# penn-graphics-research/HOT

Measured on AMD Instinct MI355X. Metric: ms per nonlinear (L-BFGS) iteration; P2G+G2P Mparticles/s; achieved HBM GB/s vs roofline, lower is better.
Workload: dtype f64; 1 GPU; C2: one 63^3-cell cube x 8 ppc (63^3 cells per GPU), fixed-corotated E=50000 nu=0.3, dx=0.01, dt=1/24, -lsolver 3 -mg_level 3 -smoother 5 -coarseSolver 2 --project --linesearch --bcproject --usecn -cneps 1e-7; particles_per_gpu=2000376, particles_total=2000376, nodes_total=267601, levels=3, parallelism=1 GPU

## Files before the change

### hot_amd/binding.py

```python
import ctypes as C
import numpy as np

_DT = {0: np.float32, 1: np.float64}


class hot_config(C.Structure):
    _fields_ = [
        ("dtype", C.c_int32), ("device", C.c_int32), ("dx", C.c_double), ("gravity", C.c_double * 3),
        ("apic_rpic_ratio", C.c_double), ("cfl", C.c_double), ("lsolver", C.c_int32), ("Ainv", C.c_int32),
        ("smoother", C.c_int32), ("coarseSolver", C.c_int32), ("levelCnt", C.c_int32), ("times", C.c_int32),
        ("levelscale", C.c_int32), ("omega", C.c_double), ("topomega", C.c_double), ("cneps", C.c_double),
        ("useCN", C.c_int32), ("project", C.c_int32), ("systemBCProject", C.c_int32), ("linesearch", C.c_int32),
        ("matrixFree", C.c_int32), ("boundaryType", C.c_int32), ("useAdaptiveHessian", C.c_int32),
        ("topDownMGS", C.c_int32), ("max_iterations", C.c_int32), ("plasticity", C.c_int32),
        ("yield_stress", C.c_double), ("snow", C.c_double * 5), ("profile", C.c_int32), ("debug_store", C.c_int32), ("useBaselineMultigrid", C.c_int32), ("gs_chain", C.c_int32), ("gs_sub_block", C.c_int32), ("shard_gs", C.c_int32), ("shard_replicated", C.c_int32), ("ls_energy_only", C.c_int32), ("linear_iteration_cap", C.c_int32), ("shard_owner", C.c_int32), ("deterministic", C.c_int32), ("reserved", C.c_int32 * 4),
    ]


class hot_collision_object(C.Structure):
    _fields_ = [("shape", C.c_int32), ("type", C.c_int32), ("p0", C.c_double * 3), ("p1", C.c_double * 3), ("friction", C.c_double),
                ("b", C.c_double * 3), ("dbdt", C.c_double * 3), ("R", C.c_double * 9), ("omega", C.c_double * 3), ("s", C.c_double), ("dsdt", C.c_double), ("lsq", C.c_double * 4)]


STICKY, SLIP, SEPARATE = 1, 2, 3
# ... 13 lines not shown
        ("iterations", C.c_int32), ("converged", C.c_int32), ("linesearch_trials", C.c_int32),
        ("linear_iterations", C.c_int32), ("vcycles", C.c_int32), ("dropped_pairs", C.c_int32),
        ("num_nodes", C.c_int32), ("num_levels", C.c_int32), ("final_scaled_residual", C.c_double),
        ("energy", C.c_double), ("ms_sort", C.c_double), ("ms_p2g", C.c_double), ("ms_begin", C.c_double),
        ("ms_hessian", C.c_double), ("ms_mg_build", C.c_double), ("ms_solve", C.c_double), ("ms_g2p", C.c_double),
        ("ms_total", C.c_double), ("comm_calls", C.c_int64), ("comm_bytes_index", C.c_int64), ("comm_bytes_data", C.c_int64), ("comm_calls_index", C.c_int64),
    ]

    def as_dict(self):
        return {k: getattr(self, k) for k, _ in self._fields_}


ABI_SYMBOLS = [
    "default_config", "create", "destroy", "last_error", "sync", "set_particles", "get_particles", "sort",
    "get_counts", "get_indexing", "p2g", "get_grid", "set_bc", "set_sticky_halfspaces", "set_collision_objects", "begin_step", "get_dv",
    "set_dv", "update_state", "get_particle_state", "residual", "project", "cn_tolerance", "build_hessian",
    "matfree_multiply", "build_mg", "get_level", "get_matrix", "get_level_nnzb", "get_prolongation", "spmv", "restrict", "prolong",
    "smooth", "vcycle", "solve", "g2p", "line_search", "should_exit", "recover_solution", "transform_residual", "compute_step", "write_partio", "write_restart", "read_restart", "set_particle_ids", "get_particle_ids", "get_stream", "set_comm", "constitutive_eval", "plasticity_eval", "advance", "calculate_dt", "advance_frame", "profile_reset", "profile_count", "profile_get", "version", "abi_version",
]
ABI_VERSION = 7


PRODUCT_ONLY_SYMBOLS = ["rccl_unique_id", "rccl_attach", "rccl_selftest", "get_level_inblock_nnzb", "copy_bandwidth",
                        "set_plasticity_classes", "get_plasticity_classes", "plasticity_eval_classes"]


class HotError(RuntimeError):
    pass


def _ptr(a):
    if a is None:
        return None
    if hasattr(a, "data_ptr"):
        return C.c_void_p(a.data_ptr())
    return C.c_void_p(a.ctypes.data)


class HotLib:
    def __init__(self, path, prefix="hot_"):
        self.path = str(path)
        self.prefix = prefix
        self.lib = C.CDLL(self.path)
        vp, i32, i64, dbl = C.c_void_p, C.c_int32, C.c_int64, C.c_double
        P = C.POINTER
        sig = {
            "default_config": (None, [P(hot_config)]),
# ... 538 lines not shown
```

### hot_amd/csrc/hot_impl.h

```cpp
#pragma once
#include "hot_ctx.h"
#include <atomic>
#include <functional>

namespace hot {

template <class T>
struct GsImg {
    static constexpr size_t hdr_elems = 2 * 64 * 9;
    static constexpr size_t cap_entries = 1340 + 1;
    static constexpr size_t per_dir = cap_entries * 9, per_block = hdr_elems + 2 * per_dir;
    static constexpr size_t idx_per_dir = 64 * 64;
};

struct GsPlan {
    enum Path {
        CHAINED,
        COLOUR,
        PAIR,
        PER_COLOUR,
        SIMPLE,
    } path;
    int sb;
    int nmerge;
    bool winv;
    bool marks;
};
struct GsBuild {
    bool winv;
    bool images;
    bool colour_lists;
};

template <class T>
__host__ __device__ inline int home_rank(const uint64_t* split, int R, int x, int y, int z, int level)
{
    using G = Geo<T>;
    const uint64_t page = G::linear_offset((x & ~3) << level, (y & ~3) << level, (z & ~3) << level) >> 12;
    int r = 0;
    while (r < R - 1 && page >= split[r]) ++r;
    return r;
}

template <class T>
struct Level {
    int n = 0;
    int id = 0;
    bool built = false;
    long long nnzb = 0;
// ... 536 lines not shown
```

### hot_amd/csrc/mg_gs.hip

```cpp
#include "hot_impl.h"

namespace hot {

#ifdef HOT_AB_KERNELS
#include "ab_src/mg_gs_ab1.hip"
#endif

template <class T, int SB>
struct GsLds {
    static constexpr int TRI = SB * (SB - 1) / 2 + 1;
    static constexpr size_t bytes = (size_t)9 * TRI * sizeof(T) + SB * 3 * sizeof(T) + 5 * SB * sizeof(int32_t);
};
template <class T>
struct GsWinv {
    static constexpr int img_elems = (9 * GsLds<T, 64>::TRI + 15) / 16 * 16;
};
template <int SB>
__device__ __forceinline__ int gs_tri_fwd(int row, int colm) { return (SB - 1) * colm - (colm * (colm - 1)) / 2 + (row - colm - 1); }
__device__ __forceinline__ int gs_tri_bwd(int row, int colm) { return (colm * (colm - 1)) / 2 + row; }
template <bool FWD>
__device__ __forceinline__ int gs_winv_idx(int row, int colm) { return FWD ? (row * (row - 1)) / 2 + colm : ((63 - row) * (62 - row)) / 2 + (63 - colm); }

template <class T>
__device__ __forceinline__ void gs_store_tri(T* tri, int TRI, int idx, const T* __restrict__ di, const T (&b)[9])
// ... 660 lines not shown
{
    const size_t i = (size_t)blockIdx.x * blockDim.x + threadIdx.x;
    if (i >= n) return;
    if constexpr (sizeof(T) == 8)
        ((unsigned long long*)x)[i] = GsUnset<double>::bits;
    else
        ((unsigned*)x)[i] = GsUnset<float>::bits;
}
struct GsPasses {
    int npass;
    int wg_begin[34];
    int block0[33];
    int sub[33];
    int color[33];
};

#ifdef HOT_GS_CLOCKS
__device__ unsigned long long gs_clk[34 * 8];
#define GS_CLK(i) \
    do { \
        const unsigned long long t_ = clock64(); \
        gclk_[i] += t_ - gt0_, gt0_ = t_; \
    } while (0)
#else
#define GS_CLK(i)
#endif
template <class T, bool FWD, int SB, bool WINV = false>
__global__ __launch_bounds__(SB * 16) void k_gs_sweep(const int32_t* __restrict__ col, const T* __restrict__ val, const uint32_t* __restrict__ ckey, const int32_t* __restrict__ gs_order,
    const int32_t* __restrict__ block_start, const T* __restrict__ diagVal, const T* __restrict__ diagBlockInv, const T* __restrict__ rhs, T* x, T* hD, GsPasses P,
    const int32_t* __restrict__ rowcnt, int* err ,
    T* unset_next ,
    const T* __restrict__ gs_w )
{
    extern __shared__ __attribute__((aligned(16))) char gs_smem[];
    constexpr int TRI = GsLds<T, SB>::TRI;
    static_assert(!WINV || SB == 64, "the inverse images are whole-block images");
#ifdef HOT_GS_CLOCKS
    unsigned long long gclk_[5] = { 0, 0, 0, 0, 0 }, gt0_ = clock64();
#endif
    constexpr int RQ = 4, NW = SB / RQ;
    auto ld3 = [&](int64_t j, T& x0, T& x1, T& x2) {
        x0 = __hip_atomic_load(x + 3 * j, __ATOMIC_RELAXED, __HIP_MEMORY_SCOPE_AGENT), x1 = __hip_atomic_load(x + 3 * j + 1, __ATOMIC_RELAXED, __HIP_MEMORY_SCOPE_AGENT),
        x2 = __hip_atomic_load(x + 3 * j + 2, __ATOMIC_RELAXED, __HIP_MEMORY_SCOPE_AGENT);
        int spins = 0;
        while (GsUnset<T>::is(x0) || GsUnset<T>::is(x1) || GsUnset<T>::is(x2)) {
            __builtin_amdgcn_s_sleep(2);
            if (++spins > (1 << 21) || ((spins & 1023) == 0 && *(volatile int*)err)) {
                *(volatile int*)err = 1;
                break;
            }
            x0 = __hip_atomic_load(x + 3 * j, __ATOMIC_RELAXED, __HIP_MEMORY_SCOPE_AGENT), x1 = __hip_atomic_load(x + 3 * j + 1, __ATOMIC_RELAXED, __HIP_MEMORY_SCOPE_AGENT),
            x2 = __hip_atomic_load(x + 3 * j + 2, __ATOMIC_RELAXED, __HIP_MEMORY_SCOPE_AGENT);
        }
    };
    T* tri = (T*)gs_smem;
    T* sv = tri + (WINV ? GsWinv<T>::img_elems : 9 * TRI);
    int32_t* nodes = (int32_t*)(sv + 3 * SB);
    const int tid = threadIdx.x, lane = tid & 63, w = tid >> 6;
    int p = 0;
    while (p + 1 < P.npass && (int)blockIdx.x >= P.wg_begin[p + 1]) ++p;
    const int b = P.block0[p] + ((int)blockIdx.x - P.wg_begin[p]);
    const int lo = P.sub[p] * SB;
    const int start = block_start[b] + lo, cnt = max(0, min(SB, block_start[b + 1] - start));
    int32_t* rng = nodes + SB;
    T* sDinv = (T*)(nodes + 5 * SB);
    T* sD = sDinv + 9 * SB;
    T* srhs = sD + 9 * SB;
    if (!WINV)
        for (int e = tid; e < 9 * TRI; e += 64 * NW) tri[e] = (T)0;
    if (tid < SB) nodes[tid] = tid < cnt ? gs_order[start + tid] : -1;
    __syncthreads();
    GS_CLK(0);
    if (WINV) {
        constexpr int IMG_BYTES = GsWinv<T>::img_elems * (int)sizeof(T);
        const char* wg = (const char*)(gs_w + ((size_t)b * 2 + (FWD ? 0 : 1)) * GsWinv<T>::img_elems);
        for (int c = w; c * 1024 < IMG_BYTES; c += NW) {
            const int off = c * 1024 + lane * 16;
            if (off < IMG_BYTES)
                __builtin_amdgcn_global_load_lds((const __attribute__((address_space(1))) void*)(wg + off), (__attribute__((address_space(3))) void*)((char*)tri + c * 1024), 16, 0, 0);
        }
    }
    for (int e = tid; e < 9 * cnt; e += 64 * NW) {
        const int64_t i = nodes[e / 9];
        sDinv[e] = diagBlockInv[9 * i + e % 9];
        if (FWD) sD[e] = diagVal[9 * i + e % 9];
    }
    for (int e = tid; e < 3 * cnt; e += 64 * NW) srhs[e] = rhs[3 * (int64_t)nodes[e / 3] + e % 3];
    if (unset_next)
        for (int e = tid; e < 3 * cnt; e += 64 * NW) gs_store_unset(unset_next + 3 * (int64_t)nodes[e / 3] + e % 3);
    T bv[RQ][9];
    int jj[RQ], node[RQ], kb2[RQ], ke[RQ];
    const bool first_sub = p == 0 || P.color[p - 1] != P.color[p];
    const bool head = FWD ? first_sub : !first_sub;
    bool late[RQ];
    const uint32_t prevkey = p > 0 ? ((uint32_t)P.color[p - 1] << 8) | (uint32_t)P.sub[p - 1] : 0xffffffffu;
    if constexpr (WINV) {
        int4 rc[RQ];
#pragma unroll
        for (int q = 0; q < RQ; ++q) {
            const int ii = w + NW * q;
            jj[q] = -1, kb2[q] = 0, ke[q] = 0, late[q] = false;
            node[q] = ii < cnt ? __builtin_amdgcn_readfirstlane(nodes[ii]) : -1;
#pragma unroll
            for (int e = 0; e < 9; ++e) bv[q][e] = (T)0;
        }
#pragma unroll
        for (int q = 0; q < RQ; ++q) rc[q] = node[q] >= 0 ? *(const int4*)(rowcnt + 4 * (int64_t)node[q]) : make_int4(0, 0, 0, 0);
#pragma unroll
        for (int q = 0; q < RQ; ++q) {
            if (node[q] < 0) continue;
            const int64_t i = node[q];
            const int kbeg = FWD ? 0 : rc[q].x + rc[q].y + 1 + rc[q].z, kend = FWD ? rc[q].x : kbeg + rc[q].w;
            kb2[q] = head ? kbeg + 64 : kbeg, ke[q] = head ? kend : kend - 64;
            const int k = head ? kbeg + lane : kend - 64 + lane;
            if (k >= kbeg && k < kend) {
                jj[q] = col[i * 125 + k];
                const T* bb = val + (i * 125 + k) * 9;
#pragma unroll
                for (int e = 0; e < 9; ++e) bv[q][e] = bb[e];
            }
        }
#pragma unroll
        for (int q = 0; q < RQ; ++q)
            if (jj[q] >= 0) {
                const uint32_t keyj = ckey[jj[q]];
                late[q] = (((keyj >> 28) << 8) | (((keyj & 127u) - 1u) / (uint32_t)SB)) == prevkey;
            }
    }
    else
#pragma unroll
    for (int q = 0; q < RQ; ++q) {
        const int ii = w + NW * q;
        jj[q] = -1, node[q] = -1, kb2[q] = 0, ke[q] = 0, late[q] = false;
#pragma unroll
        for (int e = 0; e < 9; ++e) bv[q][e] = (T)0;
        if (ii < cnt) {
            const int i = nodes[ii];
            node[q] = i;
            const int po = rowcnt[4 * i], pi = rowcnt[4 * i + 1], fi = rowcnt[4 * i + 2], fo = rowcnt[4 * i + 3];
            const int kbeg = FWD ? 0 : po + pi + 1, kend = FWD ? po + pi : po + pi + 1 + fi + fo;
            const int ibeg = FWD ? po : kbeg, iend = FWD ? po + pi : kbeg + fi;
            kb2[q] = head ? kbeg + 64 : kbeg, ke[q] = head ? kend : kend - 64;
            rng[ii] = kb2[q], rng[SB + ii] = ke[q];
            const int k = head ? kbeg + lane : kend - 64 + lane;
            if (k >= kbeg && k < kend) {
                const int j = col[(int64_t)i * 125 + k];
                const T* bb = val + ((int64_t)i * 125 + k) * 9;
#pragma unroll
                for (int e = 0; e < 9; ++e) bv[q][e] = bb[e];
                jj[q] = j;
                const uint32_t keyj = ckey[j];
                late[q] = (((keyj >> 28) << 8) | (((keyj & 127u) - 1u) / (uint32_t)SB)) == prevkey;
                if (k >= ibeg && k < iend) {
                    const int l = (int)(keyj & 127u) - 1 - lo;
                    if (l >= 0 && l < SB) {
                        if (!WINV) {
                            const int idx = FWD ? gs_tri_fwd<SB>(ii, l) : gs_tri_bwd(ii, l);
                            gs_store_tri<T>(tri, TRI, idx, diagBlockInv + 9 * (int64_t)i, bv[q]);
                        }
                        jj[q] = -1;
                    }
                }
            }
        }
    }
    __syncthreads();
    GS_CLK(1);
    auto is_late = [&](uint32_t keyj) { return (((keyj >> 28) << 8) | (((keyj & 127u) - 1u) / (uint32_t)SB)) == prevkey; };
    bool tail_late[RQ];
#pragma unroll
    for (int q = 0; q < RQ; ++q) {
        const int ii = w + NW * q;
        tail_late[q] = false;
        if (ii >= cnt) continue;
        const int i = WINV ? node[q] : nodes[ii], kt0 = WINV ? kb2[q] : rng[ii], kt1 = WINV ? ke[q] : rng[SB + ii];
        T e0 = 0, e1 = 0, e2 = 0;
        if (jj[q] >= 0 && !late[q]) {
            const int64_t j = jj[q];
            T x0, x1, x2;
            ld3(j, x0, x1, x2);
            e0 = bv[q][0] * x0 + bv[q][3] * x1 + bv[q][6] * x2;
            e1 = bv[q][1] * x0 + bv[q][4] * x1 + bv[q][7] * x2;
            e2 = bv[q][2] * x0 + bv[q][5] * x1 + bv[q][8] * x2;
        }
        bool tl = false;
        for (int k = kt0 + lane; k < kt1; k += 64) {
            const int j = col[(int64_t)i * 125 + k];
            const T* bb = val + ((int64_t)i * 125 + k) * 9;
            const uint32_t keyj = ckey[j], keyi = ckey[i];
            const int l = (int)(keyj & 127u) - 1 - lo;
            if ((keyj >> 7) == (keyi >> 7) && l >= 0 && l < SB) {
                if (!WINV) {
                    const int idx = FWD ? gs_tri_fwd<SB>(ii, l) : gs_tri_bwd(ii, l);
                    T bt[9];
#pragma unroll
                    for (int e = 0; e < 9; ++e) bt[e] = bb[e];
                    gs_store_tri<T>(tri, TRI, idx, diagBlockInv + 9 * (int64_t)i, bt);
                }
            }
            else if (is_late(keyj))
                tl = true;
            else {
                T x0, x1, x2;
                ld3(j, x0, x1, x2);
                e0 += bb[0] * x0 + bb[3] * x1 + bb[6] * x2;
                e1 += bb[1] * x0 + bb[4] * x1 + bb[7] * x2;
                e2 += bb[2] * x0 + bb[5] * x1 + bb[8] * x2;
            }
        }
        tail_late[q] = __ballot(tl) != 0ull;
        e0 = wave_sum(e0), e1 = wave_sum(e1), e2 = wave_sum(e2);
        if (lane == 0) srhs[3 * ii] -= e0, srhs[3 * ii + 1] -= e1, srhs[3 * ii + 2] -= e2;
    }
    GS_CLK(2);
    const T* val_again = val;
    asm volatile("" : "+s"(val_again));
#pragma unroll
    for (int q = 0; q < RQ; ++q) {
        const int ii = w + NW * q;
        if (ii >= cnt) continue;
        const int i = WINV ? node[q] : nodes[ii], kt0 = WINV ? kb2[q] : rng[ii], kt1 = WINV ? ke[q] : rng[SB + ii];
        T s0 = 0, s1 = 0, s2 = 0;
        if (jj[q] >= 0 && late[q]) {
            const int64_t j = jj[q];
            const T* bb = val_again + ((int64_t)i * 125 + (head ? kt0 - 64 : kt1) + lane) * 9;
            T bl[9];
#pragma unroll
            for (int e = 0; e < 9; ++e) bl[e] = bb[e];
            T x0, x1, x2;
            ld3(j, x0, x1, x2);
            s0 = bl[0] * x0 + bl[3] * x1 + bl[6] * x2;
            s1 = bl[1] * x0 + bl[4] * x1 + bl[7] * x2;
            s2 = bl[2] * x0 + bl[5] * x1 + bl[8] * x2;
        }
        if (tail_late[q]) {
            for (int k = kt0 + lane; k < kt1; k += 64) {
                const int j = col[(int64_t)i * 125 + k];
                const T* bb = val + ((int64_t)i * 125 + k) * 9;
                const uint32_t keyj = ckey[j], keyi = ckey[i];
                const int l = (int)(keyj & 127u) - 1 - lo;
                if (!((keyj >> 7) == (keyi >> 7) && l >= 0 && l < SB) && is_late(keyj)) {
                    T x0, x1, x2;
                    ld3(j, x0, x1, x2);
                    s0 += bb[0] * x0 + bb[3] * x1 + bb[6] * x2;
                    s1 += bb[1] * x0 + bb[4] * x1 + bb[7] * x2;
                    s2 += bb[2] * x0 + bb[5] * x1 + bb[8] * x2;
                }
            }
        }
        s0 = wave_sum(s0), s1 = wave_sum(s1), s2 = wave_sum(s2);
        if (lane == 0) gs_store_rhs<T>(sv, ii, sDinv + 9 * ii, srhs[3 * ii] - s0, srhs[3 * ii + 1] - s1, srhs[3 * ii + 2] - s2);
    }
    __syncthreads();
    GS_CLK(3);
#ifdef HOT_GS_CLOCKS
#define GS_CLK_OUT() \
    do { \
        GS_CLK(4); \
        if (tid == 0) \
            for (int i = 0; i < 5; ++i) atomicAdd(&gs_clk[p * 8 + i], gclk_[i]); \
        if (tid == 0) atomicAdd(&gs_clk[p * 8 + 7], 1ull); \
    } while (0)
#else
#define GS_CLK_OUT()
#endif
    if (WINV) {
        const bool cin = lane < cnt;
        const T ac0 = cin ? sv[3 * lane] : (T)0, ac1 = cin ? sv[3 * lane + 1] : (T)0, ac2 = cin ? sv[3 * lane + 2] : (T)0;
        T h0 = 0, h1 = 0, h2 = 0;
#pragma unroll
        for (int k = 0; k < 4; ++k) {
            const int rr = 4 * w + k;
            if (rr >= cnt) break;
            const bool act = FWD ? lane < rr : (lane > rr && cin);
            const int idx = act ? gs_winv_idx<FWD>(rr, lane) : TRI - 1;
            T Lw[9];
#pragma unroll
            for (int e = 0; e < 9; ++e) Lw[e] = tri[e * TRI + idx];
            T t0 = Lw[0] * ac0 + Lw[3] * ac1 + Lw[6] * ac2, t1 = Lw[1] * ac0 + Lw[4] * ac1 + Lw[7] * ac2, t2 = Lw[2] * ac0 + Lw[5] * ac1 + Lw[8] * ac2;
            t0 = wave_sum(t0), t1 = wave_sum(t1), t2 = wave_sum(t2);
            if (lane == k) h0 = sv[3 * rr] + t0, h1 = sv[3 * rr + 1] + t1, h2 = sv[3 * rr + 2] + t2;
        }
        const int me = 4 * w + lane;
        if (lane < 4 && me < cnt) {
            const int64_t i = nodes[me];
            __hip_atomic_store(x + 3 * i, h0, __ATOMIC_RELAXED, __HIP_MEMORY_SCOPE_AGENT);
            __hip_atomic_store(x + 3 * i + 1, h1, __ATOMIC_RELAXED, __HIP_MEMORY_SCOPE_AGENT);
            __hip_atomic_store(x + 3 * i + 2, h2, __ATOMIC_RELAXED, __HIP_MEMORY_SCOPE_AGENT);
            if (FWD) {
                const T* dd = sD + 9 * me;
                hD[3 * i] = dd[0] * h0 + dd[3] * h1 + dd[6] * h2, hD[3 * i + 1] = dd[1] * h0 + dd[4] * h1 + dd[7] * h2, hD[3 * i + 2] = dd[2] * h0 + dd[5] * h1 + dd[8] * h2;
            }
            else if (hD)
                hD[3 * i] += h0, hD[3 * i + 1] += h1, hD[3 * i + 2] += h2;
        }
        GS_CLK_OUT();
        return;
    }
    if (w != 0) return;
    if (cnt > 0) gs_phase_b<T, FWD, SB, true>(tri, sv, nodes, cnt, lane, diagVal, diagBlockInv, x, hD, sD);
    GS_CLK_OUT();
}

template <class T>
__global__ void k_gs_hdiff(size_t n3, T* __restrict__ h, const T* __restrict__ du)
{
    const size_t i = (size_t)blockIdx.x * blockDim.x + threadIdx.x;
    if (i < n3) h[i] -= du[i];
}
template <class T, bool DIFF = false>
__global__ __launch_bounds__(256) void k_gs_residual(const int32_t* __restrict__ col, const T* __restrict__ val, const int32_t* __restrict__ rowcnt, const T* __restrict__ h,
    const T* __restrict__ du, T* __restrict__ r, int n, const uint8_t* __restrict__ own, const uint8_t* __restrict__ owner ,
    int me, const T* __restrict__ l1e )
{
    const int lane = threadIdx.x & 63;
    const int row = xcd_block() * 4 + (threadIdx.x >> 6);
    if (row >= n || (own && !own[row])) return;
    const int nl = rowcnt[4 * row] + rowcnt[4 * row + 1];
    const int32_t* c = col + (int64_t)row * 125;
    const T* v = val + (int64_t)row * 1125;
    T s0 = 0, s1 = 0, s2 = 0;
// ... 71 lines not shown
        p.marks = L.tmp.p != nullptr;
    }
    return p;
}
template <class T>
GsBuild Ctx<T>::gs_build(const Level<T>& L) const
{
    const int max_nb = max_colour_blocks(L);
    GsBuild b{};
    b.winv = sizeof(T) == 8 && smoother_kind(L.id) == 5 && chain_allowed(*this, L, max_nb) && (cfg.gs_sub_block == 0 || cfg.gs_sub_block == 64) && L.nblocks <= 2048;
    b.images = max_nb > 256 || cfg.gs_sub_block == 32;
    b.colour_lists = !L.part && !ab_flag("HOT_GS_PAIR");
    return b;
}

template <class T>
static bool raise_gs_lds_limits(Ctx<T>& ctx)
{
    if (ctx.attr_gs_set) return false;
    HOT_HIP(hipFuncSetAttribute((const void*)k_gs_block<T, true, 64>, hipFuncAttributeMaxDynamicSharedMemorySize, (int)GsLds<T, 64>::bytes));
    HOT_HIP(hipFuncSetAttribute((const void*)k_gs_block<T, false, 64>, hipFuncAttributeMaxDynamicSharedMemorySize, (int)GsLds<T, 64>::bytes));
    HOT_HIP(hipFuncSetAttribute((const void*)k_gs_sweep<T, true, 64>, hipFuncAttributeMaxDynamicSharedMemorySize, (int)(GsLds<T, 64>::bytes + 21 * 64 * sizeof(T) + 128)));
    HOT_HIP(hipFuncSetAttribute((const void*)k_gs_sweep<T, false, 64>, hipFuncAttributeMaxDynamicSharedMemorySize, (int)(GsLds<T, 64>::bytes + 21 * 64 * sizeof(T) + 128)));
    HOT_HIP(hipFuncSetAttribute((const void*)k_gs_sweep<T, true, 64, true>, hipFuncAttributeMaxDynamicSharedMemorySize, (int)(GsLds<T, 64>::bytes + 21 * 64 * sizeof(T) + 128)));
    HOT_HIP(hipFuncSetAttribute((const void*)k_gs_sweep<T, false, 64, true>, hipFuncAttributeMaxDynamicSharedMemorySize, (int)(GsLds<T, 64>::bytes + 21 * 64 * sizeof(T) + 128)));
    ctx.attr_gs_set = true;
    return true;
}
template <class T>
struct ExchangeAfterColour {
    Ctx<T>* ctx;
    Level<T>& L;
    T* x;
    int c;
    bool on;
    ~ExchangeAfterColour()
    {
        if (on) ctx->exchange(L, x, c);
    }
};

template <class T>
void Ctx<T>::ic_smooth_dev(Level<T>& L, T* u, T* r, T* dAu)
{
    HOT_CHECK(L.ic_ready && L.split, HOT_ERR_INVALID, "coarseSolver 7: the level has no incomplete-Cholesky factor (hot_build_mg)");
    raise_gs_lds_limits(*this);
    T* y = L.tmp.p;
    for (int c = 0; c < 8; ++c) {
// ... 52 lines not shown
            if (h != 0) return;
            if (fwd)
                HOT_LAUNCH(this, lname(nm, L.id).c_str(), (k_gs_color<T, true>), nb, 64, 0, L.col.p, L.val.p, L.ckey.p, L.gs_order.p, L.gs_block_start.p, L.gs_d(), L.gs_dinv(), rhs, xx, hD, b0, nb);
            else
                HOT_LAUNCH(this, lname(nm, L.id).c_str(), (k_gs_color<T, false>), nb, 64, 0, L.col.p, L.val.p, L.ckey.p, L.gs_order.p, L.gs_block_start.p, L.gs_d(), L.gs_dinv(), rhs, xx, hD, b0, nb);
            return;
        }
#endif
        const int gs_threads = sb == 64 ? 1024 : 512;
#define HOT_GS_CASE(F, S)                                                                                                                                      \
    HOT_LAUNCH(this, lname(nm, L.id).c_str(), (k_gs_block<T, F, S>), nb, gs_threads, (GsLds<T, S>::bytes), L.col.p, L.val.p, L.ckey.p, L.gs_order.p, L.gs_block_start.p, \
        L.gs_d(), L.gs_dinv(), rhs, xx, hD, b0, h | (nmerge << 16), rc, L.gs_pad.p)
        if (fwd) {
            if (sb == 64) HOT_GS_CASE(true, 64);
            else if (sb == 32) HOT_GS_CASE(true, 32);
            else HOT_GS_CASE(true, 16);
        }
        else {
            if (sb == 64) HOT_GS_CASE(false, 64);
            else if (sb == 32) HOT_GS_CASE(false, 32);
            else HOT_GS_CASE(false, 16);
        }
#undef HOT_GS_CASE
    };
    auto per_colour_sweep = [&](bool fwd) {
        if (fwd)
            for (int c = 0; c < 8; ++c)
                for (int h = 0; h < nsub; ++h) pass(true, c, h);
        else
            for (int c = 7; c >= 0; --c)
                for (int h = nsub - 1; h >= 0; --h) pass(false, c, h);
    };

    auto pair_sweep = [&](bool fwd) {
        const T* rhs = fwd ? r : dAu;
        T* xx = fwd ? hdu : du;
        T* hD = fwd ? dAu : u;
        const char* nmT = fwd ? "gs_forward" : "gs_backward";
        const char* nmO = fwd ? "gs_forward_off" : "gs_backward_off";
        T* hsub = (!fwd && !L.part) ? hdu : (T*)nullptr;
        if (L.part) hD = fwd ? dAu : (T*)nullptr;
        for (int q = 0; q < 8; ++q) {
            const int c = fwd ? q : 7 - q;
            if (L.color_block_begin[c + 1] <= L.color_block_begin[c]) continue;
            ExchangeAfterColour<T> after{ this, L, xx, c, L.part && !rank_local };
            const auto [b0, b1] = L.colour_run(c, comm.rank, comm.size);
// ... 102 lines not shown
            int b0 = L.color_block_begin[c], nb = L.color_block_begin[c + 1] - b0;
            if (nb <= 0) return;
            P.block0[P.npass] = b0, P.sub[P.npass] = h, P.color[P.npass] = c, P.wg_begin[P.npass + 1] = P.wg_begin[P.npass] + nb;
            ++P.npass;
        };
        for (int c = 0; c < 8; ++c)
            for (int h = 0; h < nsub; ++h) add(PF, c, h);
        for (int c = 7; c >= 0; --c)
            for (int h = nsub - 1; h >= 0; --h) add(PB, c, h);
    }
    bool du_marked = false;
    auto chained_sweep = [&](bool fwd) {
        const GsPasses& P = fwd ? PF : PB;
        if (P.npass == 0) return;
        const char* nm = fwd ? "gs_forward" : "gs_backward";
        const T* rhs = fwd ? r : dAu;
        T* xx = fwd ? hdu : du;
        T* hD = fwd ? dAu : u;
        const int32_t* rc = L.rowcnt.p;
        const bool marked = fwd ? tmp_marked : du_marked;
        if (fwd) tmp_marked = false;
        if (!marked) HOT_LAUNCH(this, "gs_fill_unset", k_gs_fill_unset<T>, div_up(n3, 256), 256, 0, n3, xx);
        const int grid = P.wg_begin[P.npass];
#define HOT_GS_CASE(F, S, ...)                                                                                                                                         \
    HOT_LAUNCH(this, lname(nm, L.id).c_str(), (k_gs_sweep<T, F, S, ##__VA_ARGS__>), grid, 16 * S, (GsLds<T, S>::bytes + 21 * S * sizeof(T) + 128), L.col.p, L.val.p, L.ckey.p, L.gs_order.p, L.gs_block_start.p, \
        L.diagVal.p, L.diagBlockInv.p, rhs, xx, hD, P, rc, (int*)(hscal + 250), \
        fwd ? du : (T*)nullptr, L.gs_w.p)
        du_marked = fwd;
        if (plan.winv) {
            if (fwd)
                HOT_GS_CASE(true, 64, true);
            else
                HOT_GS_CASE(false, 64, true);
        }
        else if (fwd) {
            if (sb == 64) HOT_GS_CASE(true, 64);
            else if (sb == 32) HOT_GS_CASE(true, 32);
            else HOT_GS_CASE(true, 16);
        }
        else {
            if (sb == 64) HOT_GS_CASE(false, 64);
            else if (sb == 32) HOT_GS_CASE(false, 32);
            else HOT_GS_CASE(false, 16);
        }
#undef HOT_GS_CASE
    };
#ifdef HOT_GS_CLOCKS
    auto clk_report = [&](const char* what) {
        unsigned long long h[34 * 8];
        HOT_HIP(hipStreamSynchronize(stream));
        HOT_HIP(hipMemcpyFromSymbol(h, HIP_SYMBOL(gs_clk), sizeof(h)));
        if (h[7]) {
            fprintf(stderr, "k_gs_sweep %s level %d, clocks per workgroup [header, rows, early gathers, wait + late gathers, solve]:", what, L.id);
            for (int q = 0; q < 33 && h[q * 8 + 7]; ++q) fprintf(stderr, " | p%d(%llu wg) %.0f %.0f %.0f %.0f %.0f", q, h[q * 8 + 7], (double)h[q * 8] / h[q * 8 + 7], (double)h[q * 8 + 1] / h[q * 8 + 7], (double)h[q * 8 + 2] / h[q * 8 + 7], (double)h[q * 8 + 3] / h[q * 8 + 7], (double)h[q * 8 + 4] / h[q * 8 + 7]);
            fprintf(stderr, "\n");
        }
// ... 49 lines not shown
                if (!subtracted) HOT_LAUNCH(this, "gs_hdiff", k_gs_hdiff<T>, div_up(n3, 256), 256, 0, n3, hdu, du);
                HOT_LAUNCH(this, lname("gs_residual", L.id).c_str(), (k_gs_residual<T, true>), xcd_grid(div_up(L.n, 4)), 256, 0, L.col.p, L.val.p, L.rowcnt.p, hdu, du, r, L.n, L.mask(),
                    rank_local ? L.owner.p : (const uint8_t*)nullptr, comm.rank, (rank_local && L.l1) ? L.gsE.p : (const T*)nullptr);
            }
            else
                HOT_LAUNCH(this, lname("gs_residual", L.id).c_str(), k_gs_residual<T>, xcd_grid(div_up(L.n, 4)), 256, 0, L.col.p, L.val.p, L.rowcnt.p, hdu, du, r, L.n, L.mask(),
                    rank_local ? L.owner.p : (const uint8_t*)nullptr, comm.rank, (rank_local && L.l1) ? L.gsE.p : (const T*)nullptr);
            if (!hm) exchange(L, r, -1);
        }
        else {
            spmv_dev(L, du, dAu);
            if (level == 0 && !cfg.systemBCProject) project_dev(dAu);
            axpy(n3, (T)-1, dAu, r);
        }
    }
}

template __global__ void k_gs_fill_unset<double>(size_t n, double* x);

template struct Ctx<float>;
template struct Ctx<double>;

}
```

### include/hot_mi355x.h

```cpp
#ifndef HOT_MI355X_H
#define HOT_MI355X_H

#include <stdint.h>

#ifdef __cplusplus
extern "C" {
#endif

typedef struct hot_ctx hot_ctx;

enum hot_status {
    HOT_OK = 0,
    HOT_ERR_INVALID = -1,
    HOT_ERR_DEVICE = -2,
    HOT_ERR_CAPACITY = -3,
    HOT_ERR_NUMERIC = -4
};

typedef struct hot_config {
    int32_t dtype;
    int32_t device;
    double dx;
    double gravity[3];
    double apic_rpic_ratio;
// ... 161 lines not shown
int hot_constitutive_eval(hot_ctx*, int32_t n, const void* F , const void* mu , const void* lambda , int32_t project,
    void* psi , void* P , void* dPdF );
int hot_plasticity_eval(hot_ctx*, int32_t kind , int32_t n, void* F , void* mu , void* lambda ,
    void* Jp );

typedef struct hot_plasticity_class {
    int32_t kind;
    int32_t reserved;
    double yield_stress;
    double snow[5];
} hot_plasticity_class;
int hot_set_plasticity_classes(hot_ctx*, int32_t n, const hot_plasticity_class* classes , const int32_t* particle_class );
int hot_get_plasticity_classes(hot_ctx*, int32_t* n, hot_plasticity_class* classes , int32_t* particle_class );
int hot_plasticity_eval_classes(hot_ctx*, int32_t n, void* F , void* mu , void* lambda , void* Jp , const int32_t* cls );

int hot_write_partio(hot_ctx*, const char* path);
int hot_write_restart(hot_ctx*, const char* path);
int hot_read_restart(hot_ctx*, const char* path);

int hot_profile_reset(hot_ctx*);
int hot_profile_count(hot_ctx*, int32_t* n);
int hot_profile_get(hot_ctx*, int32_t i, char* name , int64_t* calls, double* total_ms);

const char* hot_version(void);

#ifdef __cplusplus
}
#endif
#endif
```

Before: 3.037 ms/iter.

## Split WINV Gauss-Seidel sweep into a 512-thread kernel streaming inverse images

Moves the inverse-image (WINV) Gauss-Seidel sweep into its own device function launched with 512 threads instead of 1024. Each wavefront now handles more rows. The inverse triangular image is read directly from global memory with software prefetch, replacing the copy into LDS through global_load_lds. The LDS footprint shrinks to about 24*64 elements plus index arrays, and the kernel requests a waves-per-EU occupancy target, so more workgroups can be resident per CU. In exchange, inverse-image reads go to cache and HBM instead of LDS, and each wave processes 8 rows serially.

```diff
diff --git a/hot_amd/binding.py b/hot_amd/binding.py
--- a/hot_amd/binding.py
+++ b/hot_amd/binding.py
@@ -59,7 +59,7 @@
 
 
 PRODUCT_ONLY_SYMBOLS = ["rccl_unique_id", "rccl_attach", "rccl_selftest", "get_level_inblock_nnzb", "copy_bandwidth",
-                        "set_plasticity_classes", "get_plasticity_classes", "plasticity_eval_classes"]
+                        "set_plasticity_classes", "get_plasticity_classes", "plasticity_eval_classes", "gs_winv_launch_shape"]
 
 
 class HotError(RuntimeError):
diff --git a/hot_amd/csrc/hot_impl.h b/hot_amd/csrc/hot_impl.h
--- a/hot_amd/csrc/hot_impl.h
+++ b/hot_amd/csrc/hot_impl.h
@@ -25,6 +25,11 @@
     int nmerge;
     bool winv;
     bool marks;
+};
+template <class T>
+struct GsWinvLaunch {
+    static constexpr int threads = 512;
+    static constexpr size_t lds = (size_t)24 * 64 * sizeof(T) + (64 + 64 * 64) * sizeof(int32_t);
 };
 struct GsBuild {
     bool winv;
diff --git a/hot_amd/csrc/mg_gs.hip b/hot_amd/csrc/mg_gs.hip
--- a/hot_amd/csrc/mg_gs.hip
+++ b/hot_amd/csrc/mg_gs.hip
@@ -706,39 +706,262 @@
         const unsigned long long t_ = clock64(); \
         gclk_[i] += t_ - gt0_, gt0_ = t_; \
     } while (0)
+#define GS_CLK_OUT() \
+    do { \
+        GS_CLK(4); \
+        if (tid == 0) \
+            for (int i = 0; i < 5; ++i) atomicAdd(&gs_clk[p * 8 + i], gclk_[i]); \
+        if (tid == 0) atomicAdd(&gs_clk[p * 8 + 7], 1ull); \
+    } while (0)
 #else
 #define GS_CLK(i)
-#endif
+#define GS_CLK_OUT()
+#endif
+template <class T>
+__device__ __forceinline__ void gs_ld3(const T* x, int* err, int64_t j, T& x0, T& x1, T& x2)
+{
+    x0 = __hip_atomic_load(x + 3 * j, __ATOMIC_RELAXED, __HIP_MEMORY_SCOPE_AGENT), x1 = __hip_atomic_load(x + 3 * j + 1, __ATOMIC_RELAXED, __HIP_MEMORY_SCOPE_AGENT),
+    x2 = __hip_atomic_load(x + 3 * j + 2, __ATOMIC_RELAXED, __HIP_MEMORY_SCOPE_AGENT);
+    int spins = 0;
+    while (GsUnset<T>::is(x0) || GsUnset<T>::is(x1) || GsUnset<T>::is(x2)) {
+        __builtin_amdgcn_s_sleep(2);
+        if (++spins > (1 << 21) || ((spins & 1023) == 0 && *(volatile int*)err)) {
+            *(volatile int*)err = 1;
+            break;
+        }
+        x0 = __hip_atomic_load(x + 3 * j, __ATOMIC_RELAXED, __HIP_MEMORY_SCOPE_AGENT), x1 = __hip_atomic_load(x + 3 * j + 1, __ATOMIC_RELAXED, __HIP_MEMORY_SCOPE_AGENT),
+        x2 = __hip_atomic_load(x + 3 * j + 2, __ATOMIC_RELAXED, __HIP_MEMORY_SCOPE_AGENT);
+    }
+}
+
+template <class T, bool FWD>
+__device__ __forceinline__ void gs_sweep_winv(char* smem, const int32_t* __restrict__ col, const T* __restrict__ val, const uint32_t* __restrict__ ckey, const int32_t* __restrict__ gs_order,
+    const int32_t* __restrict__ block_start, const T* __restrict__ diagVal, const T* __restrict__ diagBlockInv, const T* __restrict__ rhs, T* x, T* hD, const GsPasses& P,
+    const int32_t* __restrict__ rowcnt, int* err, T* unset_next, const T* __restrict__ gs_w)
+{
+    constexpr int SB = 64, TRI = GsLds<T, 64>::TRI;
+    constexpr int RQ = 4, NW = GsWinvLaunch<T>::threads / 64, NT = 64 * NW, RPW = SB / NW;
+    constexpr int WD = RPW < 5 ? RPW : 5;
+    static_assert(RPW % RQ == 0 && RPW >= RQ, "a wavefront streams whole rounds");
+#ifdef HOT_GS_CLOCKS
+    unsigned long long gclk_[5] = { 0, 0, 0, 0, 0 }, gt0_ = clock64();
+#endif
+    auto ld3 = [&](int64_t j, T& x0, T& x1, T& x2) { gs_ld3<T>(x, err, j, x0, x1, x2); };
+    T* sv = (T*)smem;
+    T* sDinv = sv + 3 * SB;
+    T* sD = sDinv + 9 * SB;
+    T* srhs = sD + 9 * SB;
+    int32_t* nodes = (int32_t*)(srhs + 3 * SB);
+    int32_t* sjl = nodes + SB;
+    const int tid = threadIdx.x, lane = tid & 63, w = __builtin_amdgcn_readfirstlane(tid >> 6);
+    int p = 0;
+    while (p + 1 < P.npass && (int)blockIdx.x >= P.wg_begin[p + 1]) ++p;
+    const int b = P.block0[p] + ((int)blockIdx.x - P.wg_begin[p]);
+    const int lo = P.sub[p] * SB;
+    const int start = block_start[b] + lo, cnt = max(0, min(SB, block_start[b + 1] - start));
+    if (tid < SB) nodes[tid] = tid < cnt ? gs_order[start + tid] : -1;
+    __syncthreads();
+    GS_CLK(0);
+    for (int e = tid; e < 9 * cnt; e += NT) {
+        const int64_t i = nodes[e / 9];
+        sDinv[e] = diagBlockInv[9 * i + e % 9];
+        if (FWD) sD[e] = diagVal[9 * i + e % 9];
+    }
+    for (int e = tid; e < 3 * cnt; e += NT) srhs[e] = rhs[3 * (int64_t)nodes[e / 3] + e % 3];
+    if (unset_next)
+        for (int e = tid; e < 3 * cnt; e += NT) gs_store_unset(unset_next + 3 * (int64_t)nodes[e / 3] + e % 3);
+    const bool first_sub = p == 0 || P.color[p - 1] != P.color[p];
+    const bool head = FWD ? first_sub : !first_sub;
+    const uint32_t prevkey = p > 0 ? ((uint32_t)P.color[p - 1] << 8) | (uint32_t)P.sub[p - 1] : 0xffffffffu;
+    auto is_late = [&](uint32_t keyj) { return (((keyj >> 28) << 8) | (((keyj & 127u) - 1u) / (uint32_t)SB)) == prevkey; };
+    int node[RPW], kb2[RPW], ke[RPW];
+    bool tail_late[RPW];
+#pragma unroll
+    for (int r0 = 0; r0 < RPW; r0 += RQ) {
+        T bv[RQ][9];
+        int4 rc[RQ];
+        int jj[RQ];
+        bool late[RQ];
+#pragma unroll
+        for (int q = r0; q < r0 + RQ; ++q) {
+            const int ii = w + NW * q;
+            jj[q - r0] = -1, kb2[q] = 0, ke[q] = 0, late[q - r0] = false;
+            node[q] = ii < cnt ? __builtin_amdgcn_readfirstlane(nodes[ii]) : -1;
+#pragma unroll
+            for (int e = 0; e < 9; ++e) bv[q - r0][e] = (T)0;
+        }
+#pragma unroll
+        for (int q = r0; q < r0 + RQ; ++q) rc[q - r0] = node[q] >= 0 ? *(const int4*)(rowcnt + 4 * (int64_t)node[q]) : make_int4(0, 0, 0, 0);
+#pragma unroll
+        for (int q = r0; q < r0 + RQ; ++q) {
+            if (node[q] < 0) continue;
+            const int64_t i = node[q];
+            const int4 c4 = rc[q - r0];
+            const int kbeg = FWD ? 0 : c4.x + c4.y + 1 + c4.z, kend = FWD ? c4.x : kbeg + c4.w;
+            kb2[q] = __builtin_amdgcn_readfirstlane(head ? kbeg + 64 : kbeg), ke[q] = __builtin_amdgcn_readfirstlane(head ? kend : kend - 64);
+            const int k = head ? kbeg + lane : kend - 64 + lane;
+            if (k >= kbeg && k < kend) {
+                jj[q - r0] = col[i * 125 + k];
+                const T* bb = val + (i * 125 + k) * 9;
+#pragma unroll
+                for (int e = 0; e < 9; ++e) bv[q - r0][e] = bb[e];
+            }
+        }
+#pragma unroll
+        for (int q = r0; q < r0 + RQ; ++q)
+            if (jj[q - r0] >= 0) late[q - r0] = is_late(ckey[jj[q - r0]]);
+#pragma unroll
+        for (int q = r0; q < r0 + RQ; ++q) sjl[64 * (w + NW * q) + lane] = late[q - r0] ? jj[q - r0] : -1;
+        if (r0 == 0) {
+            __syncthreads();
+            GS_CLK(1);
+        }
+#pragma unroll
+        for (int q = r0; q < r0 + RQ; ++q) {
+            const int ii = w + NW * q;
+            tail_late[q] = false;
+            if (ii >= cnt) continue;
+            int i = node[q], kt0 = kb2[q], kt1 = ke[q];
+            asm volatile("" : "+s"(i), "+s"(kt0), "+s"(kt1));
+            T e0 = 0, e1 = 0, e2 = 0;
+            if (jj[q - r0] >= 0 && !late[q - r0]) {
+                const int64_t j = jj[q - r0];
+                T x0, x1, x2;
+                ld3(j, x0, x1, x2);
+                e0 = bv[q - r0][0] * x0 + bv[q - r0][3] * x1 + bv[q - r0][6] * x2;
+                e1 = bv[q - r0][1] * x0 + bv[q - r0][4] * x1 + bv[q - r0][7] * x2;
+                e2 = bv[q - r0][2] * x0 + bv[q - r0][5] * x1 + bv[q - r0][8] * x2;
+            }
+            bool tl = false;
+            for (int k = kt0 + lane; k < kt1; k += 64) {
+                const int j = col[(int64_t)i * 125 + k];
+                const T* bb = val + ((int64_t)i * 125 + k) * 9;
+                const uint32_t keyj = ckey[j], keyi = ckey[i];
+                const int l = (int)(keyj & 127u) - 1 - lo;
+                if ((keyj >> 7) == (keyi >> 7) && l >= 0 && l < SB) continue;
+                if (is_late(keyj))
+                    tl = true;
+                else {
+                    T x0, x1, x2;
+                    ld3(j, x0, x1, x2);
+                    e0 += bb[0] * x0 + bb[3] * x1 + bb[6] * x2;
+                    e1 += bb[1] * x0 + bb[4] * x1 + bb[7] * x2;
+                    e2 += bb[2] * x0 + bb[5] * x1 + bb[8] * x2;
+                }
+            }
+            tail_late[q] = __ballot(tl) != 0ull;
+            e0 = wave_sum(e0), e1 = wave_sum(e1), e2 = wave_sum(e2);
+            if (lane == 0) srhs[3 * ii] -= e0, srhs[3 * ii + 1] -= e1, srhs[3 * ii + 2] -= e2;
+        }
+        asm volatile("" ::: "memory");
+    }
+    GS_CLK(2);
+    const T* wimg = gs_w + ((size_t)b * 2 + (FWD ? 0 : 1)) * GsWinv<T>::img_elems;
+    const bool cin = lane < cnt;
+    auto w_request = [&](int rr, T (&L)[9]) __attribute__((always_inline)) {
+        const bool act = rr < cnt && (FWD ? lane < rr : (lane > rr && cin));
+        const int idx = act ? gs_winv_idx<FWD>(rr, lane) : TRI - 1;
+#pragma unroll
+        for (int e = 0; e < 9; ++e) L[e] = wimg[e * TRI + idx];
+        asm volatile("" ::: "memory");
+    };
+    const T* val_again = val;
+    asm volatile("" : "+s"(val_again));
+#pragma unroll
+    for (int q = 0; q < RPW; ++q) {
+        const int ii = w + NW * q;
+        if (ii >= cnt) continue;
+        int i = node[q], kt0 = kb2[q], kt1 = ke[q];
+        asm volatile("" : "+s"(i), "+s"(kt0), "+s"(kt1));
+        T s0 = 0, s1 = 0, s2 = 0;
+        const int jl = sjl[64 * ii + lane];
+        if (jl >= 0) {
+            const int64_t j = jl;
+            const T* bb = val_again + ((int64_t)i * 125 + (head ? kt0 - 64 : kt1) + lane) * 9;
+            T bl[9];
+#pragma unroll
+            for (int e = 0; e < 9; ++e) bl[e] = bb[e];
+            T x0, x1, x2;
+            ld3(j, x0, x1, x2);
+            s0 = bl[0] * x0 + bl[3] * x1 + bl[6] * x2;
+            s1 = bl[1] * x0 + bl[4] * x1 + bl[7] * x2;
+            s2 = bl[2] * x0 + bl[5] * x1 + bl[8] * x2;
+        }
+        if (tail_late[q]) {
+            for (int k = kt0 + lane; k < kt1; k += 64) {
+                const int j = col[(int64_t)i * 125 + k];
+                const T* bb = val + ((int64_t)i * 125 + k) * 9;
+                const uint32_t keyj = ckey[j], keyi = ckey[i];
+                const int l = (int)(keyj & 127u) - 1 - lo;
+                if (!((keyj >> 7) == (keyi >> 7) && l >= 0 && l < SB) && is_late(keyj)) {
+                    T x0, x1, x2;
+                    ld3(j, x0, x1, x2);
+                    s0 += bb[0] * x0 + bb[3] * x1 + bb[6] * x2;
+                    s1 += bb[1] * x0 + bb[4] * x1 + bb[7] * x2;
+                    s2 += bb[2] * x0 + bb[5] * x1 + bb[8] * x2;
+                }
+            }
+        }
+        s0 = wave_sum(s0), s1 = wave_sum(s1), s2 = wave_sum(s2);
+        if (lane == 0) gs_store_rhs<T>(sv, ii, sDinv + 9 * ii, srhs[3 * ii] - s0, srhs[3 * ii + 1] - s1, srhs[3 * ii + 2] - s2);
+        if ((q + 1) % RQ == 0) asm volatile("" ::: "memory");
+    }
+    T Lw[WD][9];
+#pragma unroll
+    for (int k = 0; k < WD; ++k) w_request(RPW * w + k, Lw[k]);
+    __syncthreads();
+    GS_CLK(3);
+    const T ac0 = cin ? sv[3 * lane] : (T)0, ac1 = cin ? sv[3 * lane + 1] : (T)0, ac2 = cin ? sv[3 * lane + 2] : (T)0;
+    T h0 = 0, h1 = 0, h2 = 0;
+#pragma unroll
+    for (int k = 0; k < RPW; ++k) {
+        const int rr = RPW * w + k;
+        T(&L)[9] = Lw[k % WD];
+        T t0 = L[0] * ac0 + L[3] * ac1 + L[6] * ac2, t1 = L[1] * ac0 + L[4] * ac1 + L[7] * ac2, t2 = L[2] * ac0 + L[5] * ac1 + L[8] * ac2;
+        if (k + WD < RPW) {
+            asm volatile("" : "+v"(t0), "+v"(t1), "+v"(t2)::"memory");
+            w_request(rr + WD, L);
+        }
+        t0 = wave_sum(t0), t1 = wave_sum(t1), t2 = wave_sum(t2);
+        if (lane == k) h0 = sv[3 * rr] + t0, h1 = sv[3 * rr + 1] + t1, h2 = sv[3 * rr + 2] + t2;
+    }
+    const int me = RPW * w + lane;
+    if (lane < RPW && me < cnt) {
+        const int64_t i = nodes[me];
+        __hip_atomic_store(x + 3 * i, h0, __ATOMIC_RELAXED, __HIP_MEMORY_SCOPE_AGENT);
+        __hip_atomic_store(x + 3 * i + 1, h1, __ATOMIC_RELAXED, __HIP_MEMORY_SCOPE_AGENT);
+        __hip_atomic_store(x + 3 * i + 2, h2, __ATOMIC_RELAXED, __HIP_MEMORY_SCOPE_AGENT);
+        if (FWD) {
+            const T* dd = sD + 9 * me;
+            hD[3 * i] = dd[0] * h0 + dd[3] * h1 + dd[6] * h2, hD[3 * i + 1] = dd[1] * h0 + dd[4] * h1 + dd[7] * h2, hD[3 * i + 2] = dd[2] * h0 + dd[5] * h1 + dd[8] * h2;
+        }
+        else if (hD)
+            hD[3 * i] += h0, hD[3 * i + 1] += h1, hD[3 * i + 2] += h2;
+    }
+    GS_CLK_OUT();
+}
+
 template <class T, bool FWD, int SB, bool WINV = false>
-__global__ __launch_bounds__(SB * 16) void k_gs_sweep(const int32_t* __restrict__ col, const T* __restrict__ val, const uint32_t* __restrict__ ckey, const int32_t* __restrict__ gs_order,
+__global__ __launch_bounds__(WINV ? GsWinvLaunch<T>::threads : SB * 16) __attribute__((amdgpu_waves_per_eu(WINV ? 4 : SB / 16))) void k_gs_sweep(const int32_t* __restrict__ col, const T* __restrict__ val, const uint32_t* __restrict__ ckey, const int32_t* __restrict__ gs_order,
     const int32_t* __restrict__ block_start, const T* __restrict__ diagVal, const T* __restrict__ diagBlockInv, const T* __restrict__ rhs, T* x, T* hD, GsPasses P,
     const int32_t* __restrict__ rowcnt, int* err ,
     T* unset_next ,
     const T* __restrict__ gs_w )
 {
     extern __shared__ __attribute__((aligned(16))) char gs_smem[];
+    static_assert(!WINV || SB == 64, "the inverse images are whole-block images");
+    if constexpr (WINV) {
+        gs_sweep_winv<T, FWD>(gs_smem, col, val, ckey, gs_order, block_start, diagVal, diagBlockInv, rhs, x, hD, P, rowcnt, err, unset_next, gs_w);
+        return;
+    }
     constexpr int TRI = GsLds<T, SB>::TRI;
-    static_assert(!WINV || SB == 64, "the inverse images are whole-block images");
 #ifdef HOT_GS_CLOCKS
     unsigned long long gclk_[5] = { 0, 0, 0, 0, 0 }, gt0_ = clock64();
 #endif
     constexpr int RQ = 4, NW = SB / RQ;
-    auto ld3 = [&](int64_t j, T& x0, T& x1, T& x2) {
-        x0 = __hip_atomic_load(x + 3 * j, __ATOMIC_RELAXED, __HIP_MEMORY_SCOPE_AGENT), x1 = __hip_atomic_load(x + 3 * j + 1, __ATOMIC_RELAXED, __HIP_MEMORY_SCOPE_AGENT),
-        x2 = __hip_atomic_load(x + 3 * j + 2, __ATOMIC_RELAXED, __HIP_MEMORY_SCOPE_AGENT);
-        int spins = 0;
-        while (GsUnset<T>::is(x0) || GsUnset<T>::is(x1) || GsUnset<T>::is(x2)) {
-            __builtin_amdgcn_s_sleep(2);
-            if (++spins > (1 << 21) || ((spins & 1023) == 0 && *(volatile int*)err)) {
-                *(volatile int*)err = 1;
-                break;
-            }
-            x0 = __hip_atomic_load(x + 3 * j, __ATOMIC_RELAXED, __HIP_MEMORY_SCOPE_AGENT), x1 = __hip_atomic_load(x + 3 * j + 1, __ATOMIC_RELAXED, __HIP_MEMORY_SCOPE_AGENT),
-            x2 = __hip_atomic_load(x + 3 * j + 2, __ATOMIC_RELAXED, __HIP_MEMORY_SCOPE_AGENT);
-        }
-    };
+    auto ld3 = [&](int64_t j, T& x0, T& x1, T& x2) { gs_ld3<T>(x, err, j, x0, x1, x2); };
     T* tri = (T*)gs_smem;
-    T* sv = tri + (WINV ? GsWinv<T>::img_elems : 9 * TRI);
+    T* sv = tri + 9 * TRI;
     int32_t* nodes = (int32_t*)(sv + 3 * SB);
     const int tid = threadIdx.x, lane = tid & 63, w = tid >> 6;
     int p = 0;
@@ -750,20 +973,10 @@
     T* sDinv = (T*)(nodes + 5 * SB);
     T* sD = sDinv + 9 * SB;
     T* srhs = sD + 9 * SB;
-    if (!WINV)
-        for (int e = tid; e < 9 * TRI; e += 64 * NW) tri[e] = (T)0;
+    for (int e = tid; e < 9 * TRI; e += 64 * NW) tri[e] = (T)0;
     if (tid < SB) nodes[tid] = tid < cnt ? gs_order[start + tid] : -1;
     __syncthreads();
     GS_CLK(0);
-    if (WINV) {
-        constexpr int IMG_BYTES = GsWinv<T>::img_elems * (int)sizeof(T);
-        const char* wg = (const char*)(gs_w + ((size_t)b * 2 + (FWD ? 0 : 1)) * GsWinv<T>::img_elems);
-        for (int c = w; c * 1024 < IMG_BYTES; c += NW) {
-            const int off = c * 1024 + lane * 16;
-            if (off < IMG_BYTES)
-                __builtin_amdgcn_global_load_lds((const __attribute__((address_space(1))) void*)(wg + off), (__attribute__((address_space(3))) void*)((char*)tri + c * 1024), 16, 0, 0);
-        }
-    }
     for (int e = tid; e < 9 * cnt; e += 64 * NW) {
         const int64_t i = nodes[e / 9];
         sDinv[e] = diagBlockInv[9 * i + e % 9];
@@ -778,40 +991,6 @@
     const bool head = FWD ? first_sub : !first_sub;
     bool late[RQ];
     const uint32_t prevkey = p > 0 ? ((uint32_t)P.color[p - 1] << 8) | (uint32_t)P.sub[p - 1] : 0xffffffffu;
-    if constexpr (WINV) {
-        int4 rc[RQ];
-#pragma unroll
-        for (int q = 0; q < RQ; ++q) {
-            const int ii = w + NW * q;
-            jj[q] = -1, kb2[q] = 0, ke[q] = 0, late[q] = false;
-            node[q] = ii < cnt ? __builtin_amdgcn_readfirstlane(nodes[ii]) : -1;
-#pragma unroll
-            for (int e = 0; e < 9; ++e) bv[q][e] = (T)0;
-        }
-#pragma unroll
-        for (int q = 0; q < RQ; ++q) rc[q] = node[q] >= 0 ? *(const int4*)(rowcnt + 4 * (int64_t)node[q]) : make_int4(0, 0, 0, 0);
-#pragma unroll
-        for (int q = 0; q < RQ; ++q) {
-            if (node[q] < 0) continue;
-            const int64_t i = node[q];
-            const int kbeg = FWD ? 0 : rc[q].x + rc[q].y + 1 + rc[q].z, kend = FWD ? rc[q].x : kbeg + rc[q].w;
-            kb2[q] = head ? kbeg + 64 : kbeg, ke[q] = head ? kend : kend - 64;
-            const int k = head ? kbeg + lane : kend - 64 + lane;
-            if (k >= kbeg && k < kend) {
-                jj[q] = col[i * 125 + k];
-                const T* bb = val + (i * 125 + k) * 9;
-#pragma unroll
-                for (int e = 0; e < 9; ++e) bv[q][e] = bb[e];
-            }
-        }
-#pragma unroll
-        for (int q = 0; q < RQ; ++q)
-            if (jj[q] >= 0) {
-                const uint32_t keyj = ckey[jj[q]];
-                late[q] = (((keyj >> 28) << 8) | (((keyj & 127u) - 1u) / (uint32_t)SB)) == prevkey;
-            }
-    }
-    else
 #pragma unroll
     for (int q = 0; q < RQ; ++q) {
         const int ii = w + NW * q;
@@ -838,10 +1017,8 @@
                 if (k >= ibeg && k < iend) {
                     const int l = (int)(keyj & 127u) - 1 - lo;
                     if (l >= 0 && l < SB) {
-                        if (!WINV) {
-                            const int idx = FWD ? gs_tri_fwd<SB>(ii, l) : gs_tri_bwd(ii, l);
-                            gs_store_tri<T>(tri, TRI, idx, diagBlockInv + 9 * (int64_t)i, bv[q]);
-                        }
+                        const int idx = FWD ? gs_tri_fwd<SB>(ii, l) : gs_tri_bwd(ii, l);
+                        gs_store_tri<T>(tri, TRI, idx, diagBlockInv + 9 * (int64_t)i, bv[q]);
                         jj[q] = -1;
                     }
                 }
@@ -857,7 +1034,7 @@
         const int ii = w + NW * q;
         tail_late[q] = false;
         if (ii >= cnt) continue;
-        const int i = WINV ? node[q] : nodes[ii], kt0 = WINV ? kb2[q] : rng[ii], kt1 = WINV ? ke[q] : rng[SB + ii];
+        const int i = nodes[ii], kt0 = rng[ii], kt1 = rng[SB + ii];
         T e0 = 0, e1 = 0, e2 = 0;
         if (jj[q] >= 0 && !late[q]) {
             const int64_t j = jj[q];
@@ -874,13 +1051,11 @@
             const uint32_t keyj = ckey[j], keyi = ckey[i];
             const int l = (int)(keyj & 127u) - 1 - lo;
             if ((keyj >> 7) == (keyi >> 7) && l >= 0 && l < SB) {
-                if (!WINV) {
-                    const int idx = FWD ? gs_tri_fwd<SB>(ii, l) : gs_tri_bwd(ii, l);
-                    T bt[9];
-#pragma unroll
-                    for (int e = 0; e < 9; ++e) bt[e] = bb[e];
-                    gs_store_tri<T>(tri, TRI, idx, diagBlockInv + 9 * (int64_t)i, bt);
-                }
+                const int idx = FWD ? gs_tri_fwd<SB>(ii, l) : gs_tri_bwd(ii, l);
+                T bt[9];
+#pragma unroll
+                for (int e = 0; e < 9; ++e) bt[e] = bb[e];
+                gs_store_tri<T>(tri, TRI, idx, diagBlockInv + 9 * (int64_t)i, bt);
             }
             else if (is_late(keyj))
                 tl = true;
@@ -903,7 +1078,7 @@
     for (int q = 0; q < RQ; ++q) {
         const int ii = w + NW * q;
         if (ii >= cnt) continue;
-        const int i = WINV ? node[q] : nodes[ii], kt0 = WINV ? kb2[q] : rng[ii], kt1 = WINV ? ke[q] : rng[SB + ii];
+        const int i = nodes[ii], kt0 = rng[ii], kt1 = rng[SB + ii];
         T s0 = 0, s1 = 0, s2 = 0;
         if (jj[q] >= 0 && late[q]) {
             const int64_t j = jj[q];
@@ -937,50 +1112,6 @@
     }
     __syncthreads();
     GS_CLK(3);
-#ifdef HOT_GS_CLOCKS
-#define GS_CLK_OUT() \
-    do { \
-        GS_CLK(4); \
-        if (tid == 0) \
-            for (int i = 0; i < 5; ++i) atomicAdd(&gs_clk[p * 8 + i], gclk_[i]); \
-        if (tid == 0) atomicAdd(&gs_clk[p * 8 + 7], 1ull); \
-    } while (0)
-#else
-#define GS_CLK_OUT()
-#endif
-    if (WINV) {
-        const bool cin = lane < cnt;
-        const T ac0 = cin ? sv[3 * lane] : (T)0, ac1 = cin ? sv[3 * lane + 1] : (T)0, ac2 = cin ? sv[3 * lane + 2] : (T)0;
-        T h0 = 0, h1 = 0, h2 = 0;
-#pragma unroll
-        for (int k = 0; k < 4; ++k) {
-            const int rr = 4 * w + k;
-            if (rr >= cnt) break;
-            const bool act = FWD ? lane < rr : (lane > rr && cin);
-            const int idx = act ? gs_winv_idx<FWD>(rr, lane) : TRI - 1;
-            T Lw[9];
-#pragma unroll
-            for (int e = 0; e < 9; ++e) Lw[e] = tri[e * TRI + idx];
-            T t0 = Lw[0] * ac0 + Lw[3] * ac1 + Lw[6] * ac2, t1 = Lw[1] * ac0 + Lw[4] * ac1 + Lw[7] * ac2, t2 = Lw[2] * ac0 + Lw[5] * ac1 + Lw[8] * ac2;
-            t0 = wave_sum(t0), t1 = wave_sum(t1), t2 = wave_sum(t2);
-            if (lane == k) h0 = sv[3 * rr] + t0, h1 = sv[3 * rr + 1] + t1, h2 = sv[3 * rr + 2] + t2;
-        }
-        const int me = 4 * w + lane;
-        if (lane < 4 && me < cnt) {
-            const int64_t i = nodes[me];
-            __hip_atomic_store(x + 3 * i, h0, __ATOMIC_RELAXED, __HIP_MEMORY_SCOPE_AGENT);
-            __hip_atomic_store(x + 3 * i + 1, h1, __ATOMIC_RELAXED, __HIP_MEMORY_SCOPE_AGENT);
-            __hip_atomic_store(x + 3 * i + 2, h2, __ATOMIC_RELAXED, __HIP_MEMORY_SCOPE_AGENT);
-            if (FWD) {
-                const T* dd = sD + 9 * me;
-                hD[3 * i] = dd[0] * h0 + dd[3] * h1 + dd[6] * h2, hD[3 * i + 1] = dd[1] * h0 + dd[4] * h1 + dd[7] * h2, hD[3 * i + 2] = dd[2] * h0 + dd[5] * h1 + dd[8] * h2;
-            }
-            else if (hD)
-                hD[3 * i] += h0, hD[3 * i + 1] += h1, hD[3 * i + 2] += h2;
-        }
-        GS_CLK_OUT();
-        return;
-    }
     if (w != 0) return;
     if (cnt > 0) gs_phase_b<T, FWD, SB, true>(tri, sv, nodes, cnt, lane, diagVal, diagBlockInv, x, hD, sD);
     GS_CLK_OUT();
@@ -1098,8 +1229,7 @@
     HOT_HIP(hipFuncSetAttribute((const void*)k_gs_block<T, false, 64>, hipFuncAttributeMaxDynamicSharedMemorySize, (int)GsLds<T, 64>::bytes));
     HOT_HIP(hipFuncSetAttribute((const void*)k_gs_sweep<T, true, 64>, hipFuncAttributeMaxDynamicSharedMemorySize, (int)(GsLds<T, 64>::bytes + 21 * 64 * sizeof(T) + 128)));
     HOT_HIP(hipFuncSetAttribute((const void*)k_gs_sweep<T, false, 64>, hipFuncAttributeMaxDynamicSharedMemorySize, (int)(GsLds<T, 64>::bytes + 21 * 64 * sizeof(T) + 128)));
-    HOT_HIP(hipFuncSetAttribute((const void*)k_gs_sweep<T, true, 64, true>, hipFuncAttributeMaxDynamicSharedMemorySize, (int)(GsLds<T, 64>::bytes + 21 * 64 * sizeof(T) + 128)));
-    HOT_HIP(hipFuncSetAttribute((const void*)k_gs_sweep<T, false, 64, true>, hipFuncAttributeMaxDynamicSharedMemorySize, (int)(GsLds<T, 64>::bytes + 21 * 64 * sizeof(T) + 128)));
+    static_assert(GsWinvLaunch<T>::lds <= 64 * 1024, "k_gs_sweep<.., WINV> stays under the default dynamic-LDS limit: nothing to raise");
     ctx.attr_gs_set = true;
     return true;
 }
@@ -1198,6 +1328,7 @@
             else HOT_GS_CASE(false, 16);
         }
 #undef HOT_GS_CASE
+#undef HOT_GS_LAUNCH
     };
     auto per_colour_sweep = [&](bool fwd) {
         if (fwd)
@@ -1346,16 +1477,16 @@
         if (fwd) tmp_marked = false;
         if (!marked) HOT_LAUNCH(this, "gs_fill_unset", k_gs_fill_unset<T>, div_up(n3, 256), 256, 0, n3, xx);
         const int grid = P.wg_begin[P.npass];
-#define HOT_GS_CASE(F, S, ...)                                                                                                                                         \
-    HOT_LAUNCH(this, lname(nm, L.id).c_str(), (k_gs_sweep<T, F, S, ##__VA_ARGS__>), grid, 16 * S, (GsLds<T, S>::bytes + 21 * S * sizeof(T) + 128), L.col.p, L.val.p, L.ckey.p, L.gs_order.p, L.gs_block_start.p, \
-        L.diagVal.p, L.diagBlockInv.p, rhs, xx, hD, P, rc, (int*)(hscal + 250), \
-        fwd ? du : (T*)nullptr, L.gs_w.p)
+#define HOT_GS_LAUNCH(K, THREADS, LDS)                                                                                                                        \
+    HOT_LAUNCH(this, lname(nm, L.id).c_str(), K, grid, THREADS, LDS, L.col.p, L.val.p, L.ckey.p, L.gs_order.p, L.gs_block_start.p, L.diagVal.p, L.diagBlockInv.p, rhs, xx, \
+        hD, P, rc, (int*)(hscal + 250), fwd ? du : (T*)nullptr, L.gs_w.p)
+#define HOT_GS_CASE(F, S) HOT_GS_LAUNCH((k_gs_sweep<T, F, S>), 16 * S, (GsLds<T, S>::bytes + 21 * S * sizeof(T) + 128))
         du_marked = fwd;
         if (plan.winv) {
             if (fwd)
-                HOT_GS_CASE(true, 64, true);
+                HOT_GS_LAUNCH((k_gs_sweep<T, true, 64, true>), GsWinvLaunch<T>::threads, GsWinvLaunch<T>::lds);
             else
-                HOT_GS_CASE(false, 64, true);
+                HOT_GS_LAUNCH((k_gs_sweep<T, false, 64, true>), GsWinvLaunch<T>::threads, GsWinvLaunch<T>::lds);
         }
         else if (fwd) {
             if (sb == 64) HOT_GS_CASE(true, 64);
@@ -1451,3 +1582,11 @@
 template struct Ctx<double>;
 
 }
+
+extern "C" int hot_gs_winv_launch_shape(int32_t dtype, int32_t* threads, int32_t* lds_bytes)
+{
+    if ((dtype != 0 && dtype != 1) || !threads || !lds_bytes) return HOT_ERR_INVALID;
+    *threads = dtype ? hot::GsWinvLaunch<double>::threads : hot::GsWinvLaunch<float>::threads;
+    *lds_bytes = (int32_t)(dtype ? hot::GsWinvLaunch<double>::lds : hot::GsWinvLaunch<float>::lds);
+    return 0;
+}
diff --git a/include/hot_mi355x.h b/include/hot_mi355x.h
--- a/include/hot_mi355x.h
+++ b/include/hot_mi355x.h
@@ -207,6 +207,8 @@
 int hot_profile_count(hot_ctx*, int32_t* n);
 int hot_profile_get(hot_ctx*, int32_t i, char* name , int64_t* calls, double* total_ms);
 
+int hot_gs_winv_launch_shape(int32_t dtype, int32_t* threads, int32_t* lds_bytes);
+
 const char* hot_version(void);
 
 #ifdef __cplusplus
```

New measurement: 3.361 ms/iter. 1.11x slower.
